# skylinemusiccds/Llama.github.io

Measured on AMD Instinct MI355X. Metric: GBM train rows/sec (100 trees, depth 6) on HIGGS-11M at 1/2/4/8 MI355X, higher is better.
Workload: dtype fp32; 1 GPU; global_batch=11000000, parallelism=dp1 (row-sharded, hist all-reduce), rows=11000000, rows_per_rank=11000000, features=28, comm_bytes_per_tree=0

## Files before the change

### llama_github_io_amd/csrc/tree_kernels.hip

```cpp
#include <hip/hip_runtime.h>
#include <stdint.h>
#include <stdlib.h>
#include <string.h>

#include "abi.h"

#define NBIN 256
#define AMAX_SHARDS 64
#define NA_BIN 255
#define FTILE 32
#define BLK 1024
#define NW (BLK / 64)
#define TILE 2048
#define LEAFQ_STRIPES 16
#define LPR 8
#define RPI (BLK / LPR)

struct Node {
  int start, len, build, parent, sib ,
      dir , pad1, pad2;
};

#define NBW 32
#define GROUP_CAT 2
// ... 738 lines not shown
        float wf = 0.f;
        hist_span<PACKED, UNIT, NONA, BUF, FINE>(h, nayy, src, W, wabs, Fl, j == 0 && ftile == 0, rs, we, g, j, wf, sa,
                                                 sb, sp, srep, snb, sfine, (dbg & 2) != 0);
        wyy += (double)wf;
        since += we - rs;
        rs = we;
      }
    }
  }
  for (int t = FILT ? t0 : t1; t < t1; ++t) {
    const int node = find_node(tile_prefix, n_nodes, t);
    const Node nd = nodes[node];
    if (!nd.build) continue;
    const int r0 = nd.start + (t - tile_prefix[node]) * TILE;
    const int r1 = min(r0 + TILE, nd.start + nd.len);
    if (node != cur || (packed && since + (r1 - r0) > PACK_MAX)) {
      if (cur >= 0) flush();
      acc = node == cur;
      lds_zero64(h, packed ? HPLANE : 2 * HPLANE);
      for (int i = threadIdx.x; i < FTILE; i += blockDim.x) nayy[i] = 0.f;
      if (FILT && threadIdx.x < (int)(sizeof(Dec) / 4))
        ((int*)&spd)[threadIdx.x] = ((const int*)(pdec + nd.parent))[threadIdx.x];
      wyy = 0.0;
      lcnt = 0;
      since = 0;
      cur = node;
      cur_parent = nd.parent;
      __syncthreads();
      if (FILT) {
        flt.feat = spd.feat;
        flt.fptr = bins + bin_off(0, spd.feat, stride, N, planar);
        flt.fstride = planar ? 32 : stride;
        if (fdir) { flt.fptr = fdir; flt.fstride = 1; }
        const int jw = (spd.feat >> 2) - ftile * LPR;
        flt.jw = (jw >= 0 && jw < LPR) ? jw : -1;
        flt.dir = nd.dir;
        flt.bin = spd.bin; flt.na_left = spd.na_left; flt.is_cat = spd.is_cat;
        if (fdir) { flt.bin = 1; flt.na_left = 0; flt.is_cat = 0; }
        flt.count = ftile == 0;
      }
    }
    since += r1 - r0;
    float wf = 0.f;
    if (FILT) {
      if (pre_t != t) filt_load(flt, r0, r1, pre);
      unsigned curb[FNP];
#pragma unroll
      for (int k = 0; k < FNP; ++k) curb[k] = pre[k];
      const int nend = nd.start + nd.len;
      const int rn1 = r0 + TILE, rn2 = r0 + 2 * TILE;
      if (pre2_t == t + 1) {
#pragma unroll
        for (int k = 0; k < FNP; ++k) pre[k] = pre2[k];
        pre_t = t + 1;
      } else if (t + 1 < t1 && rn1 < nend) {
        filt_load(flt, rn1, min(rn1 + TILE, nend), pre);
        pre_t = t + 1;
      } else {
        pre_t = -1;
      }
      if (t + 2 < t1 && rn2 < nend) {
        filt_load(flt, rn2, min(rn2 + TILE, nend), pre2);
        pre2_t = t + 2;
      } else {
        pre2_t = -1;
      }
      qn = filt_append(flt, r0, r1, wq, qn, lcnt, curb);
      while (qn >= 64) {
        unsigned wdN[8];
        float yN[8], wN[8];
        wave_sync_lds();
        filt_gather<UNIT, BUF>(FL, src, W, wq, 64, lane >> 3, wdN, yN, wN);
        const int rest = qn - 64;
        wave_sync_lds();
        const int v0 = lane < rest ? wq[64 + lane] : 0, v1 = lane + 64 < rest ? wq[128 + lane] : 0;
        if (lane < rest) wq[lane] = v0;
        if (lane + 64 < rest) wq[64 + lane] = v1;
        qn = rest;
        if (np > 0) filt_atoms<PACKED, UNIT, NONA, FINE>(FL, h, nayy, np, lane >> 3, j, wdP, yP, wP, wf, sa, sb, sp);
#pragma unroll
        for (int u = 0; u < 8; ++u) { wdP[u] = wdN[u]; yP[u] = yN[u]; wP[u] = wN[u]; }
        np = 64;
      }
    }
    wyy += (double)wf;
  }
  if (cur >= 0) flush();
}

#define RW 8
template <typename P, typename TO, bool COLS>
__global__ __launch_bounds__(RW * 64) void k_hist_reduce(
    const P* __restrict__ partials, int slot_doubles, int used, const Node* __restrict__ nodes,
    const int* __restrict__ bp, const int* __restrict__ meta, int G, TO* __restrict__ out, int ostride,
    double* __restrict__ hist_next, const double* __restrict__ hist_cur, int lo_F) {
  const int node = blockIdx.y;
  if (node >= meta[0]) return;
  const Node nd = nodes[node];
  if (!nd.build) return;
  __shared__ double red[RW][64];
  const int n_tiles = meta[2];
  const int per = n_tiles > 0 ? (n_tiles + G - 1) / G : 1;
  const int t0 = bp[node], t1 = bp[node + 1];
  const int b0 = t0 / per, b1 = t1 > t0 ? (t1 - 1) / per : b0 - 1;
  const int oslot = nd.parent >= 0 ? nd.parent : 0;
  const int lane = threadIdx.x & 63, w = threadIdx.x >> 6;
  int i = (COLS ? blockIdx.x * RW + w : blockIdx.x) * 64 + lane;
  if (lo_F > 0) {
    const int F = (used - 1) / (2 * NBIN + 1), lo2 = 2 * lo_F;
    const int vb = NBIN * lo2;
    if (i >= vb + F + 1) i = used;
    else i = i < vb ? (i / lo2) * 2 * F + i % lo2 : NBIN * 2 * F + (i - vb);
  }
  const int ic = min(i, used - 1);
  double a[8] = {0.0, 0.0, 0.0, 0.0, 0.0, 0.0, 0.0, 0.0};
  constexpr int ST = COLS ? 1 : RW;
  int b = b0 + (COLS ? 0 : w);
  for (; b + 7 * ST <= b1; b += 8 * ST) {
#pragma unroll
    for (int k = 0; k < 8; ++k) a[k] += (double)partials[(size_t)(b + k * ST + node) * slot_doubles + ic];
  }
  for (; b <= b1; b += ST) a[0] += (double)partials[(size_t)(b + node) * slot_doubles + ic];
  double acc = ((a[0] + a[1]) + (a[2] + a[3])) + ((a[4] + a[5]) + (a[6] + a[7]));
  if (!COLS) {
    red[w][lane] = acc;
    __syncthreads();
    if (w != 0) return;
    acc = red[0][lane];
#pragma unroll
    for (int k = 1; k < RW; ++k) acc += red[k][lane];
  }
  if (i >= used) return;
  if (out) out[(size_t)oslot * ostride + i] = (TO)acc;
  if (hist_next) {
    hist_next[(size_t)node * slot_doubles + i] = acc;
    if (nd.sib >= 0)
      hist_next[(size_t)nd.sib * slot_doubles + i] = hist_cur[(size_t)nd.parent * slot_doubles + i] - acc;
  }
}

struct Derive {
  const void* recv;
  int f32, E;
  const double* prev;
  const Node* nodes;
};

__device__ __forceinline__ double add_mul_rn(double a, double x, double y) {
#pragma clang fp contract(off)
  return a + x * y;
}

struct HistRead {
  const double* slot;
  const void* recv;
  const double* pv;
  size_t rb;
  int f32, build, derive;
  __device__ __forceinline__ double operator()(size_t i) const {
    if (!derive) return slot[i];
    const double r = f32 ? (double)((const float*)recv)[rb + i] : ((const double*)recv)[rb + i];
    return build ? r : pv[i] - r;
  }
};
#define GBINS 1024
__device__ void split_find_group(const HistRead& hv, int node, int f, int gg, int hs, int FL,
// ... 1726 lines not shown
  __shared__ unsigned short acc[64][256];
  const int tid = threadIdx.x;
  const long long row = (long long)blockIdx.x * 256 + tid;
  for (int k = 0; k < nslot; ++k) acc[k][tid] = 0;
  if (row >= N) return;
  for (int pl = 0; pl < planes; ++pl) {
    const uint4* src = (const uint4*)(master + ((size_t)pl * (size_t)N + (size_t)row) * 32);
    const uint4 v0 = src[0], v1 = src[1];
    const unsigned wd[8] = {v0.x, v0.y, v0.z, v0.w, v1.x, v1.y, v1.z, v1.w};
#pragma unroll
    for (int c = 0; c < 32; ++c) {
      const int sl = cslot[pl * 32 + c];
      if (sl < 0) continue;
      const unsigned b = (wd[c >> 2] >> (8 * (c & 3))) & 0xFFu;
      if (b == NA_BIN) acc[sl][tid] = 0x8000;
      else acc[sl][tid] = (unsigned short)(acc[sl][tid] + b);
    }
  }
  const int p16 = (nslot + 15) / 16;
  for (int q = 0; q < p16; ++q) {
    unsigned w[8];
#pragma unroll
    for (int i = 0; i < 8; ++i) {
      unsigned lo = 0, hi = 0;
      const int s0 = q * 16 + 2 * i, s1 = s0 + 1;
      if (s0 < nslot) { lo = acc[s0][tid]; lo = (lo & 0x8000u) ? 1023u : lo; }
      if (s1 < nslot) { hi = acc[s1][tid]; hi = (hi & 0x8000u) ? 1023u : hi; }
      w[i] = lo | (hi << 16);
    }
    uint4* dst = (uint4*)(fine + ((size_t)q * (size_t)N + (size_t)row) * 16);
    dst[0] = make_uint4(w[0], w[1], w[2], w[3]);
    dst[1] = make_uint4(w[4], w[5], w[6], w[7]);
  }
}

static int hist_dbg() {
  const char* e = getenv("H2O_HIST_DBG");
  return e ? atoi(e) : 0;
}

template <bool FILT, bool PACKED, bool UNIT, bool NONA, bool BUF>
static void launch_hist4(dim3 grid, size_t lds, hipStream_t s, const void* bins, int stride, const void* aw,
                         const void* ay, const void* nodes, const void* tile_prefix, const void* meta, int F,
                         void* partials, int slot_doubles, const void* qs, const void* pdec, void* nl_out, int f32,
                         long long N, int planar, int lgw, const void* nbins_f, const void* fine_f, const void* fdir) {
#define H2O_HB(FINE_)                                                                                              \
  hipLaunchKernelGGL((k_hist_build<FILT, PACKED, UNIT, NONA, BUF, FINE_>), grid, dim3(BLK), lds, s,               \
                     (const uint8_t*)bins, stride, (const float*)aw, (const float*)ay, (const Node*)nodes,         \
                     (const int*)tile_prefix, (const int*)meta, F, (double*)partials, slot_doubles, (const double*)qs, \
                     (const Dec*)pdec, (int*)nl_out, f32, N, planar, lgw, (const int*)nbins_f, (const int*)fine_f,  \
                     (const uint8_t*)fdir, hist_dbg())
  if (fine_f) H2O_HB(true); else H2O_HB(false);
#undef H2O_HB
}

template <bool PACKED, bool UNIT>
static void launch_hist(dim3 grid, size_t lds, hipStream_t s, const void* bins, int stride, const void* aw,
                        const void* ay, const void* nodes, const void* tile_prefix, const void* meta, int F,
                        void* partials, int slot_doubles, const void* qs, const void* pdec, void* nl_out, int f32,
                        long long N, int planar, const void* nbins_f, const void* fine_f, const void* fdir) {
  const bool nona = (planar >> 1) & 1;
  planar &= 1;
  const int rowb = planar ? 32 : stride;
  const unsigned long long bytes = (unsigned long long)N * (unsigned long long)rowb;
  int lgw = -1;
  for (int k = 0; k < 12; ++k) if (rowb == (1 << k)) lgw = k;
  const char* e_buf = getenv("H2O_HIST_BUF");
  const bool buf = lgw >= 0 && bytes < (1ull << 32) && (unsigned long long)N * 4ull < (1ull << 32) &&
                   !(e_buf && strcmp(e_buf, "0") == 0);
#define H2O_HIST_CASE(F_, N_, B_) \
  launch_hist4<F_, PACKED, UNIT, N_, B_>(grid, lds, s, bins, stride, aw, ay, nodes, tile_prefix, meta, F, partials, \
                                          slot_doubles, qs, pdec, nl_out, f32, N, planar, lgw, nbins_f, fine_f, fdir)
  const bool filt = pdec != nullptr;
  if (filt) {
    if (nona) { if (buf) H2O_HIST_CASE(true, true, true); else H2O_HIST_CASE(true, true, false); }
    else { if (buf) H2O_HIST_CASE(true, false, true); else H2O_HIST_CASE(true, false, false); }
  } else {
    if (nona) { if (buf) H2O_HIST_CASE(false, true, true); else H2O_HIST_CASE(false, true, false); }
    else { if (buf) H2O_HIST_CASE(false, false, true); else H2O_HIST_CASE(false, false, false); }
  }
#undef H2O_HIST_CASE
}

template <typename P, typename TO>
static void reduce_launch(const void* partials, int slot_doubles, int used, const void* nodes, const void* bp,
                          const void* meta, int cap, int grid, void* out, int ostride, void* hist_next,
                          const void* hist_cur, int lo_F, hipStream_t s) {
  const int F = (used - 1) / (2 * NBIN + 1);
  if (lo_F >= F) lo_F = 0;
  const int n = lo_F > 0 ? NBIN * 2 * lo_F + F + 1 : used;
  if (cap >= 16 && !getenv("H2O_REDUCE_SPLIT")) {
    const int gx = (n + 64 * RW - 1) / (64 * RW);
    hipLaunchKernelGGL((k_hist_reduce<P, TO, true>), dim3(gx, cap), dim3(RW * 64), 0, s, (const P*)partials,
                       slot_doubles, used, (const Node*)nodes, (const int*)bp, (const int*)meta, grid, (TO*)out,
                       ostride, (double*)hist_next, (const double*)hist_cur, lo_F);
    return;
  }
  const int gx = (n + 63) / 64;
  hipLaunchKernelGGL((k_hist_reduce<P, TO, false>), dim3(gx, cap), dim3(RW * 64), 0, s, (const P*)partials, slot_doubles,
                     used, (const Node*)nodes, (const int*)bp, (const int*)meta, grid, (TO*)out, ostride,
                     (double*)hist_next, (const double*)hist_cur, lo_F);
}

extern "C" {

int h2o_abi_version() { return H2O_ABI_VERSION; }

int h2o_tree_sizes(int* out) {
  out[7] = AMAX_SHARDS;
  out[8] = LEAFQ_STRIPES;
  out[0] = sizeof(Node); out[1] = sizeof(Dec); out[2] = sizeof(Cand); out[3] = TILE; out[4] = FTILE;
  out[5] = HIST_LDS_BYTES + HIST_LDS_TAIL;
  out[6] = BLK;
  return 0;
}

int h2o_hist_build(const void* bins, int stride, const void* aw, const void* ay, const void* nodes,
                   const void* tile_prefix, const void* meta, int F, void* partials, int slot_doubles, const void* qs,
                   int grid, int packed, const void* pdec, void* nl_out, int f32, long long N, int planar,
                   const void* nbins_f, const void* fine_f, int nft_lim, const void* fdir, hipStream_t s) {
  int nft = (F + FTILE - 1) / FTILE;
  if (nft_lim > 0 && nft_lim < nft) nft = nft_lim;
  const char* e_repl = getenv("H2O_HIST_REPL");
  const char* e_fine = getenv("H2O_HIST_FINE");
  const bool repl = !e_repl || strcmp(e_repl, "0") != 0;
  const bool fine = e_fine && strcmp(e_fine, "1") == 0;
  if (!repl) nbins_f = nullptr;
  if (!fine) fine_f = nullptr;
  const size_t lds = (packed ? HIST_LDS_BYTES - HPLANE * 8 : HIST_LDS_BYTES) + HIST_LDS_TAIL;
  const dim3 gr(grid, nft);
  if (packed && aw == nullptr)
    launch_hist<true, true>(gr, lds, s, bins, stride, aw, ay, nodes, tile_prefix, meta, F, partials, slot_doubles, qs, pdec, nl_out, f32, N, planar, nbins_f, fine_f, fdir);
  else if (packed) launch_hist<true, false>(gr, lds, s, bins, stride, aw, ay, nodes, tile_prefix, meta, F, partials, slot_doubles, qs, pdec, nl_out, f32, N, planar, nbins_f, fine_f, fdir);
  else launch_hist<false, false>(gr, lds, s, bins, stride, aw, ay, nodes, tile_prefix, meta, F, partials, slot_doubles, qs, pdec, nl_out, f32, N, planar, nbins_f, fine_f, fdir);
  return (int)hipGetLastError();
}


int h2o_fine16_build(const void* master, int planes, long long N, const void* cslot, int nslot, void* fine,
                     hipStream_t s) {
  if (nslot < 1 || nslot > 64 || planes < 1 || N <= 0) return (int)hipErrorInvalidValue;
  hipLaunchKernelGGL(k_fine16_build, dim3((unsigned)((N + 255) / 256)), dim3(256), 0, s, (const uint8_t*)master, planes,
                     N, (const int*)cslot, nslot, (unsigned short*)fine);
  return (int)hipGetLastError();
}

int h2o_hist_root16(const void* fine, int planes, const void* aw, const void* ay, long long N, const void* meta,
                    const void* fcol, const void* fnc, int F, void* partials, int slot_doubles, const void* qs, int grid,
                    int f32, hipStream_t s) {
  if (planes < 1 || grid < 1 || N <= 0) return (int)hipErrorInvalidValue;
  const dim3 gr(grid, planes);
  if (aw == nullptr)
    hipLaunchKernelGGL((k_hist_root16<true>), gr, dim3(BLK), R16_LDS, s, (const unsigned*)fine, (const float*)aw,
                       (const float*)ay, N, (const int*)meta, (const int*)fcol, (const int*)fnc, F, (double*)partials,
                       slot_doubles, (const double*)qs, f32);
  else
    hipLaunchKernelGGL((k_hist_root16<false>), gr, dim3(BLK), R16_LDS, s, (const unsigned*)fine, (const float*)aw,
                       (const float*)ay, N, (const int*)meta, (const int*)fcol, (const int*)fnc, F, (double*)partials,
                       slot_doubles, (const double*)qs, f32);
  return (int)hipGetLastError();
}

int h2o_hist_reduce(const void* partials, int slot_doubles, int used, const void* nodes, const void* bp,
                    const void* meta, int cap, int grid, void* out, void* hist_next, const void* hist_cur,
                    int f32, int out_f32, int ostride, int lo_F, hipStream_t s) {
  if (ostride <= 0) ostride = slot_doubles;
  if (f32 && out_f32)
    reduce_launch<float, float>(partials, slot_doubles, used, nodes, bp, meta, cap, grid, out, ostride, hist_next, hist_cur, lo_F, s);
  else if (f32)
    reduce_launch<float, double>(partials, slot_doubles, used, nodes, bp, meta, cap, grid, out, ostride, hist_next, hist_cur, lo_F, s);
  else if (out_f32)
    reduce_launch<double, float>(partials, slot_doubles, used, nodes, bp, meta, cap, grid, out, ostride, hist_next, hist_cur, lo_F, s);
  else
    reduce_launch<double, double>(partials, slot_doubles, used, nodes, bp, meta, cap, grid, out, ostride, hist_next, hist_cur, lo_F, s);
  return (int)hipGetLastError();
}

int h2o_leaf_values(const void* leafsum, int n, int log_link, double scale, double kclamp, double mx, double lam,
                    double l1, void* out,
                    hipStream_t s) {
  hipLaunchKernelGGL(k_leaf_values, dim3((n + 255) / 256), dim3(256), 0, s, (const double*)leafsum, n, log_link,
                     scale, kclamp, mx, lam, l1, (float*)out);
  return (int)hipGetLastError();
}

static int split_find_launch(void* hist, int slot_doubles, const void* meta, int cap, int F, const void* nbins_f,
                             const void* iscat_f, const void* mono_f, const SplitParams& p, int level, void* cand,
                             void* root_w, const void* edges, int adapt_nb, int f0, int FL, Derive dv, hipStream_t s) {
  if (F <= 0 || cap <= 0) return 0;
  if (FL < F) return (int)hipErrorInvalidValue;
  if (p.gcat)
    hipLaunchKernelGGL(k_split_find<true>, dim3(cap, F), dim3(256), 0, s, (double*)hist, slot_doubles,
                       (const int*)meta, F, (const int*)nbins_f, (const int*)iscat_f, (const int*)mono_f, p, level,
                       (Cand*)cand, (double*)root_w, (const float*)edges, adapt_nb, f0, FL, dv);
  else
    hipLaunchKernelGGL(k_split_find<false>, dim3(cap, F), dim3(256), 0, s, (double*)hist, slot_doubles,
                       (const int*)meta, F, (const int*)nbins_f, (const int*)iscat_f, (const int*)mono_f, p, level,
                       (Cand*)cand, (double*)root_w, (const float*)edges, adapt_nb, f0, FL, dv);
  return (int)hipGetLastError();
}

int h2o_split_find(const void* hist, int slot_doubles, const void* meta, int cap, int F, const void* nbins_f,
                   const void* iscat_f, const void* mono_f, double min_w, double msi, double lambda_, double alpha,
                   double gamma, int mode, int random_split, unsigned long long seed, int level, void* cand,
                   void* root_w, const void* edges, int adapt_nb, int hist_type, int f0, int FL, hipStream_t s) {
  SplitParams p;
  p.min_w = min_w; p.min_split_improvement = msi; p.lambda = lambda_; p.alpha = alpha; p.gamma = gamma;
  p.mode = mode; p.random_split = random_split; p.seed = seed; p.hist_type = hist_type; p.fcut = 0;
  p.vrange = nullptr; p.hprev = nullptr; p.pdec = nullptr; p.rnodes = nullptr; p.fgroup = nullptr; p.edges_all = nullptr;
  p.range_on = 0; p.pad_r = 0; p.gcat = nullptr;
  return split_find_launch((void*)hist, slot_doubles, meta, cap, F, nbins_f, iscat_f, mono_f, p, level, cand, root_w,
                           edges, adapt_nb, f0, FL, Derive{nullptr, 0, 0, nullptr, nullptr}, s);
}
// ... 575 lines not shown
```

### llama_github_io_amd/ops/_native.py

```python
from __future__ import annotations

import ctypes
import os
import threading

import torch

from .. import build_native

_lock = threading.Lock()
_hip = None
_rt = None

c_int, c_ll, c_ull, c_double, c_void_p = ctypes.c_int, ctypes.c_longlong, ctypes.c_ulonglong, ctypes.c_double, ctypes.c_void_p

_HIP_SIGS = {
    "h2o_tree_sizes": [c_void_p],
    "h2o_tree_plan_size": [],
    "h2o_tree_root": [c_void_p, c_void_p],
    "h2o_tree_level": [c_void_p, c_int, c_int, c_void_p],
    "h2o_tree_find": [c_void_p, c_int, c_void_p],
    "h2o_tree_grow": [c_void_p, c_int, c_int, c_void_p],
    "h2o_hist_pack": [c_void_p, c_int, c_int, c_int, c_int, c_int, c_void_p, c_int, c_void_p],
    "h2o_tree_dist": [c_void_p, c_void_p],
    "h2o_rccl_load": [ctypes.c_char_p],
    "h2o_rccl_version": [],
    "h2o_rccl_unique_id": [c_void_p],
    "h2o_rccl_id_bytes": [],
    "h2o_rccl_init": [c_void_p, c_int, c_void_p, c_int],
    "h2o_rccl_destroy": [c_void_p, c_int],
    "h2o_rccl_coll": [c_void_p, c_int, c_void_p, c_void_p, c_ll, c_int, c_void_p],
    "h2o_tree_all": [c_void_p, c_void_p],
    "h2o_tree_leaves": [c_void_p, c_void_p],
    "h2o_hist_build": [c_void_p, c_int, c_void_p, c_void_p, c_void_p, c_void_p, c_void_p, c_int, c_void_p, c_int, c_void_p,
                       c_int, c_int, c_void_p, c_void_p, c_int, c_ll, c_int, c_void_p, c_void_p, c_int, c_void_p,
                       c_void_p],
    "h2o_split_find": [c_void_p, c_int, c_void_p, c_int, c_int, c_void_p, c_void_p, c_void_p, c_double, c_double,
                       c_double, c_double, c_double, c_int, c_int, c_ull, c_int, c_void_p, c_void_p, c_void_p, c_int,
                       c_int, c_int, c_int, c_void_p],
    "h2o_split_reduce": [c_void_p, c_void_p, c_int, c_int, c_void_p, c_int, c_ull, c_int, c_void_p, c_void_p, c_void_p,
                         c_int, c_void_p],
    "h2o_ic_next": [c_void_p] * 6 + [c_int, c_void_p, c_int, c_void_p],
    "h2o_plan": [c_void_p] * 14 + [c_int, c_int, c_double, c_int, c_int, c_void_p],
    "h2o_ranges": [c_void_p] * 6,
    "h2o_zero_hist": [c_void_p, c_void_p, c_void_p, c_int, c_int, c_void_p],
    "h2o_route": [c_void_p] * 6 + [c_int] + [c_void_p] * 10 + [c_int, c_ll, c_int, c_int, c_void_p, c_void_p, c_void_p],
    "h2o_leaf_assign": [c_void_p, c_int, c_ll, c_void_p, c_int, c_void_p, c_void_p, c_void_p, c_void_p, c_void_p, c_int,
                        c_void_p, c_int, c_int, c_void_p],
    "h2o_bin_assign": [c_void_p, c_ll, c_int, c_int, c_void_p, c_int, c_void_p, c_void_p, c_void_p, c_int, c_void_p,
                       c_void_p],
    "h2o_amax": [c_void_p, c_ll, c_void_p, c_void_p],
    "h2o_kmeans_mfma_shape": [c_int, c_int, c_void_p],
    "h2o_kmeans_mfma_grid": [c_int, c_int],
    "h2o_kmeans_mfma": [c_void_p, c_ll, c_int, c_void_p, c_int, c_void_p, c_void_p, c_void_p, c_void_p, c_int, c_void_p],
    "h2o_kmeans_update": [c_void_p, c_int, c_int, c_int, c_void_p, c_void_p, c_void_p, c_void_p, c_void_p],
    "h2o_qscale": [c_void_p, c_void_p, c_void_p, c_ll, c_int, c_void_p],
    "h2o_score_hist": [c_void_p, c_void_p, c_void_p, c_ll, c_int, c_void_p, c_void_p, c_void_p, c_void_p],
    "h2o_snap_copy": [c_void_p, c_void_p, c_ll, c_void_p],
    "h2o_fine16_build": [c_void_p, c_int, c_ll, c_void_p, c_int, c_void_p, c_void_p],
    "h2o_host_dev_ptr": [c_void_p, c_void_p],
    "h2o_hist_reduce": [c_void_p, c_int, c_int, c_void_p, c_void_p, c_void_p, c_int, c_int, c_void_p, c_void_p,
                        c_void_p, c_int, c_int, c_int, c_int, c_void_p],
    "h2o_leaf_values": [c_void_p, c_int, c_int, c_double, c_double, c_double, c_double, c_double, c_void_p, c_void_p],
    "h2o_gbm_step": [c_ll, c_ll, c_int, c_void_p, c_void_p, c_void_p, c_void_p, c_void_p, ctypes.c_float, c_ull,
                     ctypes.c_float, c_void_p, c_void_p, c_int, c_void_p],
    "h2o_add_leaf": [c_ll, c_void_p, c_int, c_void_p, c_void_p, c_void_p],
    "h2o_predict": [c_void_p, c_ll, c_int] + [c_void_p] * 11 + [c_int, c_void_p, c_void_p, c_void_p],
}


ABI_VERSION = 14


def _check_abi(lib, name: str) -> None:
    fn = getattr(lib, "h2o_abi_version", None)
    got = fn() if fn is not None else -1
    if got != ABI_VERSION:
        raise RuntimeError(f"{name}: native ABI version {got} != expected {ABI_VERSION}; rebuild with "
                           "`python -m llama_github_io_amd.build_native --force`")


def _bind(lib, sigs):
    for name, args in sigs.items():
        fn = getattr(lib, name, None)
        if fn is None:
            continue
        fn.argtypes = args
        fn.restype = c_int
    return lib


def register_hip_signatures(sigs: dict) -> None:
    _HIP_SIGS.update(sigs)
    if _hip is not None:
        _bind(_hip, sigs)


def hip():
    global _hip
    if _hip is None:
        with _lock:
# ... 38 lines not shown
```

### llama_github_io_amd/ops/tree.py

```python
from __future__ import annotations

import ctypes
import math
import os
from dataclasses import dataclass, field

import numpy as np
import torch

from . import _native as nat
from ..parallel import collectives as coll

NBIN = 256
NA_BIN = 255
MAX_DATA_BINS = 255
FTILE = 32
AMAX_SHARDS = 64

NODE_DT = np.dtype([("start", "<i4"), ("len", "<i4"), ("build", "<i4"), ("parent", "<i4"), ("sib", "<i4"),
                    ("dir", "<i4"), ("p1", "<i4"), ("p2", "<i4")])
NBW = 32
DEC_DT = np.dtype([("feat", "<i4"), ("bin", "<i4"), ("na_left", "<i4"), ("is_cat", "<i4"), ("bits", "<u4", (NBW,)),
                   ("gain", "<f8"), ("wl", "<f8"), ("wr", "<f8"), ("predl", "<f4"), ("predr", "<f4")])
CAND_BYTES = 184
# ... 964 lines not shown
        b, F = self.master, self.F
        if b.numel() == 0:
            return True
        hit = torch.zeros((), dtype=torch.bool, device=b.device)
        step = 1 << 24
        if self.planar:
            for pl in range(b.shape[0]):
                nf = min(32, F - 32 * pl)
                if nf <= 0:
                    break
                for r0 in range(0, b.shape[1], step):
                    hit |= (b[pl, r0:r0 + step, :nf] == NA_BIN).any()
        else:
            for r0 in range(0, b.shape[0], step):
                hit |= (b[r0:r0 + step, :F] == NA_BIN).any()
        return not bool(hit)

    def _edges_ptr(self):
        if self.p.edges is None or not self.p.adapt_nbins:
            return 0
        if getattr(self, "_edges_dev", None) is None:
            self._edges_dev = torch.as_tensor(np.asarray(self.p.edges, dtype=np.float32), device=self.master.device).contiguous()
        return self._edges_dev.data_ptr()

    def _planes(self, aux: torch.Tensor, soa: bool) -> torch.Tensor:
        if soa:
            assert aux.shape == (4, self.N) and aux.dtype == torch.float32 and aux.is_contiguous()
            return aux
        assert aux.shape == (self.N, 4) and aux.dtype == torch.float32
        if self._soa is None:
            self._soa = torch.empty(4, self.N, dtype=torch.float32, device=self.dev)
        self._soa.copy_(aux.t())
        return self._soa

    def build(self, aux_static: torch.Tensor, feat_ok: torch.Tensor | None = None, k_cols: int = 0, seed: int = 0,
              leaf_fn=None, amax_bits: torch.Tensor | None = None, packed: bool | int = False, leaf_native=None,
              soa: bool = False, unit: bool = False, num_plane: int = 2):
        if not hasattr(self, "_plan"):
            self._plan = self._make_plan()
        planes = self._planes(aux_static, soa)
        lib, P = self.lib, self._plan
        s = nat.stream_ptr(self.dev)
        P.aux = planes.data_ptr()
        P.unit = int(bool(unit))
        P.num_plane = int(num_plane) if soa else 2
        if not unit:
            for i in range(2):
                if self.bufs[i]["w"] is None:
                    self.bufs[i]["w"] = torch.empty(self.N, dtype=torch.float32, device=self.dev)
                P.bw[i] = self.bufs[i]["w"].data_ptr()
        P.compute_amax = int(amax_bits is None)
        P.amax_bits = (self.amax_bits if amax_bits is None else amax_bits).data_ptr()
        P.feat_ok = (self.feat_ok_all if feat_ok is None else feat_ok).data_ptr()
        P.k_cols, P.packed, P.seed = _level_k(k_cols, 0), (2 if packed == 2 else int(bool(packed))), int(seed) & _M64
        for d in range(_MAXL):
            P.kc_level[d] = _level_k(k_cols, d) if isinstance(k_cols, (list, tuple)) else 0
        P.grid = self.grid * (self.hist_bpc if packed else 1)
        P.leaf_native = int(leaf_native is not None)
        if leaf_native is not None:
            lg, scale, kclamp, mx = leaf_native[:4]
            lam, l1 = (tuple(leaf_native[4:6]) + (0.0, 0.0))[:2]
            P.log_link, P.scale, P.kclamp, P.mx = int(lg), float(scale), float(kclamp), float(mx)
            P.leaf_lam, P.leaf_l1 = float(lam), float(l1)
        ref = ctypes.byref(P)
        if not self.dist_mode:
            if self._graph_replay(P, k_cols):
                pass
            else:
                nat.check(lib.h2o_tree_all(ref, s), "tree_all")
        else:
            rc = lib.h2o_tree_dist(ref, s)
            err = getattr(self.transport, "error", None)
            if err is not None:
                self.transport.error = None
                raise RuntimeError(f"tree collective failed: {err}") from err
            nat.check(rc, "tree_dist")
            if isinstance(self.transport, _native_comm_cls()):
                coll.add_stats(*self.comm_per_tree())
        if leaf_native is None and leaf_fn is not None:
            vals = leaf_fn(self.leafsum)
            self.av["leafval"].view(torch.float32)[: vals.numel()].copy_(vals.to(torch.float32))
        return self._snapshot()

    def _seed_used(self, P, k_cols) -> bool:
        ht = int(self.p.hist_type)
        return (bool(P.k_cols) or any(int(v) for v in P.kc_level) or bool(P.random_split)
                or (bool(P.edges) and ht in (HT_RANDOM, HT_ROUND_ROBIN)))

    def _graph_replay(self, P, k_cols) -> bool:
        if self.dev.type != "cuda" or os.environ.get("H2O_TREE_GRAPH", "1") == "0" or self.__dict__.get("_graph_off"):
            return False
        seed = P.seed
        if not self._seed_used(P, k_cols):
            P.seed = 0
        sig = bytes(P)
        P.seed = seed
        cache = self.__dict__.setdefault("_graphs", {})
        g = cache.get(sig)
        if g is None:
            misses = self.__dict__.get("_graph_misses", 0) + 1
            self._graph_misses = misses
            if misses > _GRAPH_CACHE:
                self._graph_off = True
                cache.clear()
                return False
            g = torch.cuda.CUDAGraph()
            try:
                with torch.cuda.graph(g, capture_error_mode="thread_local"):
                    rc = self.lib.h2o_tree_all(ctypes.byref(P), nat.stream_ptr(self.dev))
            except Exception:
                self._graph_off = True
                cache.clear()
                return False
            nat.check(rc, "tree_all (capture)")
            if len(cache) >= _GRAPH_CACHE:
                cache.pop(next(iter(cache)))
            cache[sig] = g
        else:
            self._graph_misses = 0
        g.replay()
        return True

    def _snapshot(self):
        if not self._pinned_pool and self.history and self._snap_wait:
            self._decoded.extend(self._pop(1))
        host = self._pinned_pool.pop() if self._pinned_pool else torch.empty(self.arena.numel(), dtype=torch.uint8,
                                                                               pin_memory=True)
        dptr = self._snap_dev_ptr(host) if self.dev.type == "cuda" and _SNAP_KERNEL else 0
        if dptr:
            nat.call("h2o_snap_copy", self.arena.data_ptr(), dptr, self.arena.numel(), nat.stream_ptr(self.dev))
        else:
            host.copy_(self.arena, non_blocking=True)
        ev = self._event_pool.pop() if self._event_pool else torch.cuda.Event()
        ev.record()
        self.history.append((host, ev))
        return len(self.history) - 1

    def _snap_dev_ptr(self, host: torch.Tensor) -> int:
        cache = self.__dict__.setdefault("_dev_ptrs", {})
        hp = host.data_ptr()
        if hp not in cache:
            out = ctypes.c_ulonglong(0)
            rc = nat.hip().h2o_host_dev_ptr(ctypes.c_void_p(hp), ctypes.byref(out))
            cache[hp] = int(out.value) if rc == 0 and host.is_pinned() and out.value % 16 == 0 else 0
        return cache[hp]

    def leaf_values_view(self) -> torch.Tensor:
        return self.av["leafval"].view(torch.float32)

    def pop_levels(self, ready_only: bool = False) -> list:
        out, self._decoded = self._decoded, []
        return out + self._pop(None, ready_only)

    def _pop(self, limit, ready_only: bool = False) -> list:
        out = []
        while self.history and (limit is None or len(out) < limit):
            host, ev = self.history[0]
            if ready_only and not ev.query():
                break
            ev.synchronize()
            self.history.pop(0)
            hn = host.numpy()
            o = self._off["rootw"][0]
            out.append(self._decode(hn, float(hn[o:o + 8].view(np.float64)[0])))
            self._pinned_pool.append(host)
            self._event_pool.append(ev)
# ... 127 lines not shown
```

Before: 218.0 million rows/s.

## Add streaming filtered histogram kernel with per-wave LDS ring and prefetch

Adds a new histogram kernel for the filtered (child-node) path when rows are packed into 16 or 32 bytes and all features fit in one tile. Each wave prefetches the next tile's rows into registers while it processes the current one. It applies the parent split predicate in registers and compacts the selected rows into a per-wave LDS ring buffer, then runs the atomic histogram updates in batches of 64. This is meant to hide global-load latency and avoid the separate queue/gather path, at the cost of more LDS per block (the reported LDS size now takes the larger of the two layouts) and more register pressure from the prefetch buffers. A launch counter and an environment switch are also added.

```diff
diff --git a/llama_github_io_amd/csrc/tree_kernels.hip b/llama_github_io_amd/csrc/tree_kernels.hip
--- a/llama_github_io_amd/csrc/tree_kernels.hip
+++ b/llama_github_io_amd/csrc/tree_kernels.hip
@@ -844,6 +844,175 @@
         for (int u = 0; u < 8; ++u) { wdP[u] = wdN[u]; yP[u] = yN[u]; wP[u] = wN[u]; }
         np = 64;
       }
+    }
+    wyy += (double)wf;
+  }
+  if (cur >= 0) flush();
+}
+
+__device__ __forceinline__ int row_byte(uint4 v0, uint4 v1, int f);
+__device__ __forceinline__ unsigned row_word(uint4 v0, uint4 v1, int f);
+#define FS_SLOTS 128
+#define FS_RING_BYTES(stride, weighted) ((BLK / 64) * FS_SLOTS * ((stride) + 4 + ((weighted) ? 4 : 0)))
+#define FS_LDS_BYTES(stride, weighted) (HPLANE * 8 + FTILE * 4 + 64 * 8 + FS_RING_BYTES(stride, weighted))
+
+template <bool UNIT, int NV>
+__device__ __forceinline__ void fs_load(const uint8_t* __restrict__ bins, const float* __restrict__ ay,
+                                        const float* __restrict__ aw, int r0, int r1, int p, uint4& v0, uint4& v1,
+                                        float& y, float& w) {
+  const int lane = threadIdx.x & 63, wv = threadIdx.x >> 6;
+  const int row = min(r0 + wv * WROWS + p * 64 + lane, r1 - 1);
+  const uint4* s4 = (const uint4*)(bins + (size_t)row * (NV * 16));
+  v0 = s4[0];
+  v1 = NV > 1 ? s4[1] : make_uint4(0u, 0u, 0u, 0u);
+  y = ay[row];
+  w = (!UNIT && aw) ? aw[row] : 1.f;
+}
+
+template <bool UNIT, int NV>
+__device__ __forceinline__ void fs_read(const uint4* ringb, const float* ringy, const float* ringw, int head, int g8,
+                                        int wc, unsigned (&wd)[8], float (&yv)[8], float (&wv)[8]) {
+#pragma unroll
+  for (int u = 0; u < 8; ++u) {
+    const int slot = (head + g8 + 8 * u) & (FS_SLOTS - 1);
+    wd[u] = ((const unsigned*)ringb)[slot * (NV * 4) + wc];
+    yv[u] = ringy[slot];
+    if (!UNIT) wv[u] = ringw[slot];
+  }
+}
+
+template <bool UNIT, bool NONA, int NV>
+__global__ __launch_bounds__(BLK) void k_hist_filt_stream(
+    const uint8_t* __restrict__ bins ,
+    const float* __restrict__ aw , const float* __restrict__ ay ,
+    const Node* __restrict__ nodes, const int* __restrict__ tile_prefix,
+    const int* __restrict__ meta , int F ,
+    double* __restrict__ partials, int slot_doubles, const double* __restrict__ qs, const Dec* __restrict__ pdec,
+    int* __restrict__ nl_out, int f32, long long N, const int* __restrict__ nbins_f,
+    int dbg ) {
+  constexpr int W = NV * 4;
+  extern __shared__ __attribute__((aligned(16))) long long smem64[];
+  long long* h = smem64;
+  float* nayy = (float*)(smem64 + HPLANE);
+  double* red = (double*)(nayy + FTILE);
+  const int lane = threadIdx.x & 63, wv = threadIdx.x >> 6;
+  uint4* ring0 = (uint4*)(red + 64);
+  uint4* ringb = ring0 + wv * (FS_SLOTS * NV);
+  float* ringy = (float*)(ring0 + NW * FS_SLOTS * NV) + wv * FS_SLOTS;
+  float* ringw = ringy + NW * FS_SLOTS;
+
+  const int n_nodes = meta[0], n_tiles = meta[2];
+  if (n_nodes <= 0 || n_tiles <= 0) return;
+  const int per = (n_tiles + gridDim.x - 1) / gridDim.x;
+  const int t0 = blockIdx.x * per, t1 = min(n_tiles, t0 + per);
+  if (t0 >= t1) return;
+  const int j = threadIdx.x % LPR;
+  const float sa = (float)qs[10], sb = (float)qs[12], sp = (float)qs[4];
+  const HistSrc src = make_src((const unsigned*)bins, aw, ay, N, W, 0);
+  __shared__ int srep[FTILE], snb[FTILE], sfine[FTILE];
+  if (threadIdx.x < FTILE) {
+    const int fg = threadIdx.x;
+    const int nb = (NONA && nbins_f && fg < F) ? nbins_f[fg] : 0;
+    srep[threadIdx.x] = (nb > 0 && nb * 4 <= NA_BIN) ? 4 : (nb > 0 && nb * 2 <= NA_BIN) ? 2 : 1;
+    snb[threadIdx.x] = nb;
+    sfine[threadIdx.x] = 0;
+  }
+  __syncthreads();
+
+  __shared__ Dec spd;
+  RowFilter flt{&spd, bins, NV * 16, 0, -1, 0, 0, 0, 0, true};
+  int lcnt = 0;
+  int cur = -1, since = 0, cur_parent = -1;
+  uint4 p0[FNP], p1[FNP];
+  float py[FNP], pw[FNP];
+  int pre_t = -1;
+  int qn = 0, head = 0;
+  bool acc = false;
+  double wyy = 0.0;
+  const FiltLane FL = filt_lane<true, UNIT, false>(src, W, j, F, lane >> 3, j, j == 0, srep, snb, sfine);
+  const bool atoms = !(dbg & 2);
+  auto batch = [&](int n, float& wf) {
+    unsigned wd[8];
+    float yv[8], wv8[8];
+    wave_sync_lds();
+    fs_read<UNIT, NV>(ringb, ringy, ringw, head, lane >> 3, FL.wc, wd, yv, wv8);
+    wave_sync_lds();
+    head = (head + n) & (FS_SLOTS - 1);
+    qn -= n;
+    if (atoms) filt_atoms<true, UNIT, NONA, false>(FL, h, nayy, n, lane >> 3, j, wd, yv, wv8, wf, sa, sb, sp);
+  };
+  auto drain = [&]() {
+    float wf2 = 0.f;
+    if (qn > 0) batch(qn, wf2);
+    wyy += (double)wf2;
+  };
+  auto flush = [&]() {
+    drain();
+    if (dbg & 1) return;
+    double v[4] = {wyy, (double)lcnt, 0, 0};
+    block_sum4(v, red);
+    __syncthreads();
+    const size_t so = (size_t)(blockIdx.x + cur) * slot_doubles;
+    flush_partial(h, nayy, v[0], 0, F, f32 ? (double*)((float*)partials + so) : partials + so, qs, true, acc,
+                  f32 != 0, srep, snb, sfine);
+    if (threadIdx.x == 0 && v[1] != 0.0) atomicAdd(nl_out + cur_parent, (int)v[1]);
+    __syncthreads();
+  };
+  const unsigned long long below = (1ull << lane) - 1ull;
+  for (int t = t0; t < t1; ++t) {
+    const int node = find_node(tile_prefix, n_nodes, t);
+    const Node nd = nodes[node];
+    if (!nd.build) continue;
+    const int r0 = nd.start + (t - tile_prefix[node]) * TILE;
+    const int r1 = min(r0 + TILE, nd.start + nd.len);
+    if (node != cur || since + (r1 - r0) > PACK_MAX) {
+      if (cur >= 0) flush();
+      acc = node == cur;
+      lds_zero64(h, HPLANE);
+      for (int i = threadIdx.x; i < FTILE; i += blockDim.x) nayy[i] = 0.f;
+      if (threadIdx.x < (int)(sizeof(Dec) / 4))
+        ((int*)&spd)[threadIdx.x] = ((const int*)(pdec + nd.parent))[threadIdx.x];
+      wyy = 0.0;
+      lcnt = 0;
+      since = 0;
+      cur = node;
+      cur_parent = nd.parent;
+      __syncthreads();
+      flt.feat = spd.feat;
+      flt.dir = nd.dir;
+      flt.bin = spd.bin; flt.na_left = spd.na_left; flt.is_cat = spd.is_cat;
+    }
+    since += r1 - r0;
+    if (pre_t != t) {
+#pragma unroll
+      for (int p = 0; p < FNP; ++p) fs_load<UNIT, NV>(bins, ay, aw, r0, r1, p, p0[p], p1[p], py[p], pw[p]);
+    }
+    const int nend = nd.start + nd.len, rn1 = r0 + TILE;
+    const bool more = t + 1 < t1 && rn1 < nend;
+    pre_t = more ? t + 1 : -1;
+    float wf = 0.f;
+    const bool grp = flt.is_cat == GROUP_CAT;
+#pragma unroll
+    for (int p = 0; p < FNP; ++p) {
+      const int row = r0 + wv * WROWS + p * 64 + lane;
+      bool sl = false;
+      if (row < r1) {
+        const unsigned key = grp ? row_word(p0[p], p1[p], flt.feat) : (unsigned)row_byte(p0[p], p1[p], flt.feat);
+        const bool gl = flt.left(key);
+        lcnt += gl ? 1 : 0;
+        sl = (gl ? 0 : 1) == flt.dir;
+      }
+      const unsigned long long m = __ballot(sl);
+      if (sl) {
+        const int slot = (head + qn + __popcll(m & below)) & (FS_SLOTS - 1);
+        ringb[slot * NV] = p0[p];
+        if (NV > 1) ringb[slot * NV + 1] = p1[p];
+        ringy[slot] = py[p];
+        if (!UNIT) ringw[slot] = pw[p];
+      }
+      qn += __popcll(m);
+      if (more) fs_load<UNIT, NV>(bins, ay, aw, rn1, min(rn1 + TILE, nend), p, p0[p], p1[p], py[p], pw[p]);
+      if (qn >= 64) batch(64, wf);
     }
     wyy += (double)wf;
   }
@@ -2736,6 +2905,29 @@
 #undef H2O_HIST_CASE
 }
 
+static bool filt_stream_on() {
+  const char* e = getenv("H2O_FILT_STREAM");
+  return !(e && strcmp(e, "0") == 0);
+}
+static int g_filt_stream_launches = 0;
+
+template <bool UNIT>
+static void launch_filt_stream(int grid, hipStream_t s, const void* bins, int stride, const void* aw, const void* ay,
+                               const void* nodes, const void* tile_prefix, const void* meta, int F, void* partials,
+                               int slot_doubles, const void* qs, const void* pdec, void* nl_out, int f32, long long N,
+                               bool nona, const void* nbins_f) {
+  const size_t lds = FS_LDS_BYTES(stride, !UNIT);
+#define H2O_FS(N_, NV_)                                                                                            \
+  hipLaunchKernelGGL((k_hist_filt_stream<UNIT, N_, NV_>), dim3(grid), dim3(BLK), lds, s, (const uint8_t*)bins,     \
+                     (const float*)aw, (const float*)ay, (const Node*)nodes, (const int*)tile_prefix,              \
+                     (const int*)meta, F, (double*)partials, slot_doubles, (const double*)qs, (const Dec*)pdec,    \
+                     (int*)nl_out, f32, N, (const int*)nbins_f, hist_dbg())
+  if (stride == 32) { if (nona) H2O_FS(true, 2); else H2O_FS(false, 2); }
+  else { if (nona) H2O_FS(true, 1); else H2O_FS(false, 1); }
+#undef H2O_FS
+  __atomic_fetch_add(&g_filt_stream_launches, 1, __ATOMIC_RELAXED);
+}
+
 template <typename P, typename TO>
 static void reduce_launch(const void* partials, int slot_doubles, int used, const void* nodes, const void* bp,
                           const void* meta, int cap, int grid, void* out, int ostride, void* hist_next,
@@ -2764,10 +2956,13 @@
   out[7] = AMAX_SHARDS;
   out[8] = LEAFQ_STRIPES;
   out[0] = sizeof(Node); out[1] = sizeof(Dec); out[2] = sizeof(Cand); out[3] = TILE; out[4] = FTILE;
-  out[5] = HIST_LDS_BYTES + HIST_LDS_TAIL;
+  const int lds_queue = HIST_LDS_BYTES + HIST_LDS_TAIL, lds_stream = FS_LDS_BYTES(32, true);
+  out[5] = lds_stream > lds_queue ? lds_stream : lds_queue;
   out[6] = BLK;
   return 0;
 }
+
+int h2o_filt_stream_launches() { return __atomic_load_n(&g_filt_stream_launches, __ATOMIC_RELAXED); }
 
 int h2o_hist_build(const void* bins, int stride, const void* aw, const void* ay, const void* nodes,
                    const void* tile_prefix, const void* meta, int F, void* partials, int slot_doubles, const void* qs,
@@ -2783,6 +2978,15 @@
   if (!fine) fine_f = nullptr;
   const size_t lds = (packed ? HIST_LDS_BYTES - HPLANE * 8 : HIST_LDS_BYTES) + HIST_LDS_TAIL;
   const dim3 gr(grid, nft);
+  if (pdec && packed && !(planar & 1) && !fdir && !fine_f && (stride == 16 || stride == 32) && F <= stride &&
+      nft == 1 && ((uintptr_t)bins & 15) == 0 && filt_stream_on()) {
+    const bool nona = (planar >> 1) & 1;
+    if (aw == nullptr)
+      launch_filt_stream<true>(grid, s, bins, stride, aw, ay, nodes, tile_prefix, meta, F, partials, slot_doubles, qs, pdec, nl_out, f32, N, nona, nbins_f);
+    else
+      launch_filt_stream<false>(grid, s, bins, stride, aw, ay, nodes, tile_prefix, meta, F, partials, slot_doubles, qs, pdec, nl_out, f32, N, nona, nbins_f);
+    return (int)hipGetLastError();
+  }
   if (packed && aw == nullptr)
     launch_hist<true, true>(gr, lds, s, bins, stride, aw, ay, nodes, tile_prefix, meta, F, partials, slot_doubles, qs, pdec, nl_out, f32, N, planar, nbins_f, fine_f, fdir);
   else if (packed) launch_hist<true, false>(gr, lds, s, bins, stride, aw, ay, nodes, tile_prefix, meta, F, partials, slot_doubles, qs, pdec, nl_out, f32, N, planar, nbins_f, fine_f, fdir);
diff --git a/llama_github_io_amd/ops/_native.py b/llama_github_io_amd/ops/_native.py
--- a/llama_github_io_amd/ops/_native.py
+++ b/llama_github_io_amd/ops/_native.py
@@ -17,6 +17,7 @@
 _HIP_SIGS = {
     "h2o_tree_sizes": [c_void_p],
     "h2o_tree_plan_size": [],
+    "h2o_filt_stream_launches": [],
     "h2o_tree_root": [c_void_p, c_void_p],
     "h2o_tree_level": [c_void_p, c_int, c_int, c_void_p],
     "h2o_tree_find": [c_void_p, c_int, c_void_p],
diff --git a/llama_github_io_amd/ops/tree.py b/llama_github_io_amd/ops/tree.py
--- a/llama_github_io_amd/ops/tree.py
+++ b/llama_github_io_amd/ops/tree.py
@@ -1070,6 +1070,9 @@
             self.av["leafval"].view(torch.float32)[: vals.numel()].copy_(vals.to(torch.float32))
         return self._snapshot()
 
+    def filt_stream_launches(self) -> int:
+        return int(self.lib.h2o_filt_stream_launches())
+
     def _seed_used(self, P, k_cols) -> bool:
         ht = int(self.p.hist_type)
         return (bool(P.k_cols) or any(int(v) for v in P.kc_level) or bool(P.random_split)
```

Measured after the change: 219.2 million rows/s (median of 4 runs). About the same (+0.6%).
